# TUMFTM/RadarGNN

Measured on AMD Instinct MI355X. Metric: radar frames/sec (graph-build + GNN fwd), higher is better.
Workload: dtype f32 (dense layers: fp32 operands split into 2 f16 terms after an exact power-of-two pre-scale, 3 f16 MFMA products per fp32 product, fp32 accumulate -- more accurate than fp32 MFMA against float64, tests/test_gpu_f16x2.py; RGNN_NO_F16X2=1 selects 3 bf16 terms / 6 products, RGNN_LINEAR_FP32=1 v_mfma_; 1 GPU; C2: per GPU 64 RadarScenes-shaped frames x 3000 pts, radius graph r=1.0, node feats [rcs,velocity_vector,time_index,degree], edge feats [relative_position], 4-layer MPNNConv [224,224,128,64] + emb MLPs + both heads, train-mode BatchNorm, max aggr; frames_per_gpu=64, points_per_gpu=192000, edges_per_gpu=799078, ranks_in_process_group=1

## Files before the change

include/rgnn.h:

```cpp
#ifndef RGNN_H
#define RGNN_H

#include <stdint.h>

#ifdef __cplusplus
extern "C" {
#endif

typedef void* rgnn_stream_t;

#define RGNN_OK 0
#define RGNN_ERR_INVALID_ARGUMENT (-1)
#define RGNN_ERR_LAUNCH (-2)
#define RGNN_ERR_UNSUPPORTED (-3)

#define RGNN_STATUS_KNN_TOO_FEW_POINTS 1
#define RGNN_STATUS_DOT_PRODUCT 2
#define RGNN_STATUS_TIME_INDEX_OVERFLOW 4
#define RGNN_STATUS_EDGE_COUNT_CHANGED 8
#define RGNN_STATUS_NOT_SYMMETRIC 16
#define RGNN_STATUS_SPLITK_TIMEOUT 32
#define RGNN_STATUS_GT_OBJECT_TOO_LARGE 64
#define RGNN_STATUS_GT_DEGENERATE_OBJECT 128
#define RGNN_STATUS_PREPROCESS_BAD_ROW 256
// ... 144 lines not shown
  const float* residual; int64_t ldr;
  float* out; int64_t ldo;
  int64_t m; int32_t n;
  int32_t relu_out;
  float* col_stats;
  const int32_t* row_index;
  const int64_t* m_dev;
  int32_t accumulate;
  int32_t gather_only;
  const int32_t* residual_index;
  const void* W_planes;
  int32_t w_planes_kp;
  void* splitk_ws;
  int64_t splitk_ws_bytes;
  const float* a1_scale_shift;
  int32_t a1_relu;
  int32_t relu_from_col;
  const void* W_planes_f16;
  const float* a1_bound;
  const float* a2_bound;
  float* out_absmax;
  const int32_t* a1_panel_segment;
} rgnn_linear_args;
#define RGNN_BOUND_SLOTS 256
enum { RGNN_LINEAR_PATH_OTHER = 0, RGNN_LINEAR_PATH_DMA_BF16X3 = 1, RGNN_LINEAR_PATH_DMA_F16X2 = 2 };
int32_t rgnn_linear_fwd_path(const rgnn_linear_args* args );
int64_t rgnn_linear_planes_f16_bytes(int32_t n, int32_t k);
int rgnn_linear_split_weights_f16(const float* W1, const float* W2, int64_t ldw, int32_t w_split, int32_t n, int32_t k,
                                  void* planes , rgnn_stream_t stream);
int32_t rgnn_linear_fwd_fuses_a1_affine(const rgnn_linear_args* args );
enum { RGNN_LINEAR_FAMILY_NONE = 0, RGNN_LINEAR_FAMILY_TINY = 1, RGNN_LINEAR_FAMILY_FP32 = 2, RGNN_LINEAR_FAMILY_X3 = 3,
       RGNN_LINEAR_FAMILY_DMA = 4 };
void rgnn_linear_fwd_plan(const rgnn_linear_args* args , int32_t out[8] );
int64_t rgnn_linear_splitk_ws_bytes(void);
int64_t rgnn_linear_stat_panels(int64_t m);
int32_t rgnn_linear_planes_kp(int32_t k);
int rgnn_linear_split_weights(const float* W1, const float* W2, int64_t ldw, int32_t w_split, int32_t n, int32_t k,
                              void* planes , rgnn_stream_t stream);
int rgnn_linear_fwd(const rgnn_linear_args* args , rgnn_stream_t stream);

int32_t rgnn_embed3_supported(int32_t k0, int32_t n1, int32_t n2, int32_t n3);
int rgnn_embed3(const float* x, int64_t ldx, int32_t k0, const float* W1, int64_t ldw1, const float* b1, int32_t n1,
                const void* W2_planes_f16, const float* b2, int32_t n2, const void* W3_planes_f16, const float* b3, int32_t n3,
                int32_t relu3, int64_t m, float* out, int64_t ldo, float* out_absmax, rgnn_stream_t stream);
int rgnn_tiny_mlp2(const float* A, int64_t lda, int32_t k0, const int32_t* row_index , int64_t m,
                   const float* W1, int64_t ldw1, const float* b1, int32_t n1, int32_t relu1, const float* W2, int64_t ldw2,
                   const float* b2, int32_t n2, int32_t relu2, float* out, int64_t ldo, rgnn_stream_t stream);

int rgnn_batchnorm_finalize(const float* col_stats, int64_t panels, int64_t m, int32_t n, const float* gamma,
                            const float* beta, float* running_mean, float* running_var,
                            int64_t* num_batches_tracked, int32_t training, float momentum, float eps,
                            float* scale_shift , rgnn_stream_t stream);
int rgnn_batchnorm_finalize_parts(const float* stats_a, int64_t panels_a, const int64_t* rows_a ,
                                  const float* stats_b, int64_t panels_b, const int64_t* rows_b ,
                                  int64_t m, int32_t n, const float* gamma, const float* beta, float* running_mean,
                                  float* running_var, int64_t* num_batches_tracked, int32_t training, float momentum,
                                  float eps, float* scale_shift , rgnn_stream_t stream);
int rgnn_batchnorm_finalize_bound(const float* stats_a, int64_t panels_a, const int64_t* rows_a ,
                                  const float* stats_b, int64_t panels_b, const int64_t* rows_b ,
                                  int64_t m, int32_t n, const float* gamma, const float* beta, float* running_mean,
                                  float* running_var, int64_t* num_batches_tracked, int32_t training, float momentum,
                                  float eps, float* scale_shift , const float* in_bound, float* out_bound,
                                  rgnn_stream_t stream);
int rgnn_batchnorm_segments(const float* x, int64_t ldx, const int64_t* seg_ptr , int64_t n_seg, int32_t n,
                            const float* gamma, const float* beta, float* running_mean, float* running_var,
                            int64_t* num_batches_tracked, float momentum, float eps, double* seg_sums, float* table,
// ... 261 lines not shown
```

radargnn_amd/_lib.py:

```python
from __future__ import annotations

import ctypes as C
import os

import torch

_HERE = os.path.dirname(os.path.abspath(__file__))
LIB_PATH = os.environ.get("RGNN_LIB") or os.path.join(_HERE, "librgnn.so")

c_i32, c_i64, c_f32, c_f64, c_vp = C.c_int32, C.c_int64, C.c_float, C.c_double, C.c_void_p


class RgnnGrid(C.Structure):
    _fields_ = [("X", c_vp), ("dim", c_i32), ("n", c_i64), ("frame_ptr", c_vp), ("n_frames", c_i64),
                ("ws", c_vp), ("ws_bytes", c_i64)]


class RgnnLinearArgs(C.Structure):
    _fields_ = [("A1", c_vp), ("lda1", c_i64), ("k1", c_i32),
                ("A2", c_vp), ("lda2", c_i64), ("k2", c_i32),
                ("W1", c_vp), ("W2", c_vp), ("ldw", c_i64), ("w_split", c_i32),
                ("bias1", c_vp), ("bias2", c_vp),
                ("residual", c_vp), ("ldr", c_i64),
                ("out", c_vp), ("ldo", c_i64),
# ... 29 lines not shown
    "rgnn_radius_rows_commit": (c_i32, [c_vp, c_i64, c_i64, c_vp, c_vp, c_vp, c_vp, c_vp]),
    "rgnn_knn_graph": (c_i32, [C.POINTER(RgnnGrid), c_i32, c_vp, c_vp, c_vp, c_vp]),
    "rgnn_knn_graph_attrs": (c_i32, [C.POINTER(RgnnGrid), c_i32, c_vp, c_vp, c_vp, c_vp, c_i32, c_vp, c_vp]),
    "rgnn_knn_graph_frames": (c_i32, [C.POINTER(RgnnGrid), c_i32, c_i64, c_vp, c_vp, c_vp, c_vp, c_i32, c_vp, c_vp]),
    "rgnn_knn_degree_from_csr": (c_i32, [c_vp, c_vp, c_vp, c_vp, c_i64, c_i32, c_vp, c_vp]),
    "rgnn_undirected_degree_preset": (c_i32, [c_vp, c_vp, c_i64, c_vp, c_vp]),
    "rgnn_grid_cell_order": (c_i32, [C.POINTER(RgnnGrid), c_vp, c_vp]),
    "rgnn_undirected_degree": (c_i32, [c_vp, c_vp, c_i64, c_vp, c_vp, c_vp]),
    "rgnn_csr_by_target_tmp_bytes": (c_i64, [c_i64, c_i64]),
    "rgnn_invert_permutation": (c_i32, [c_vp, c_i64, c_vp, c_vp]),
    "rgnn_source_rowptr": (c_i32, [c_vp, c_i64, c_i64, c_vp, c_vp, c_vp, c_vp]),
    "rgnn_csr_by_target": (c_i32, [c_vp, c_i64, c_i64, c_vp, c_vp, c_vp, c_vp, c_vp, c_vp]),
    "rgnn_csr_by_target_unordered": (c_i32, [c_vp, c_i64, c_i64, c_vp, c_vp, c_vp, c_vp, c_vp, c_vp]),
    "rgnn_csr_by_target_frames": (c_i32, [c_vp, c_i64, c_i64, c_i64, c_vp, c_i64, c_i64, c_vp, c_vp, c_vp, c_vp, c_vp, c_vp, c_vp, c_vp]),
    "rgnn_csr_by_target_symmetric": (c_i32, [c_vp, c_vp, c_i64, c_i64, c_vp, c_vp, c_vp, c_vp, c_vp, c_vp, c_vp]),
    "rgnn_embed3_supported": (c_i32, [c_i32, c_i32, c_i32, c_i32]),
    "rgnn_embed3": (c_i32, [c_vp, c_i64, c_i32, c_vp, c_i64, c_vp, c_i32, c_vp, c_vp, c_i32, c_vp, c_vp, c_i32, c_i32, c_i64, c_vp, c_i64,
                            c_vp, c_vp]),
    "rgnn_csr_by_target_symmetric_own": (c_i32, [c_vp, c_vp, c_i64, c_i64, c_vp, c_vp, c_vp, c_vp, c_vp, c_vp, c_vp]),
    "rgnn_edge_features": (c_i32, [c_vp, c_vp, c_vp, c_i64, C.POINTER(c_i32), c_i32, c_i32, c_vp, c_i32, c_vp, c_vp]),
    "rgnn_edge_features_reversed": (c_i32, [c_vp, c_vp, c_vp, c_i64, c_vp, c_i64, C.POINTER(c_i32), c_i32, c_i32, c_vp, c_i32, c_vp, c_vp]),
    "rgnn_node_features": (c_i32, [c_vp, c_vp, c_vp, c_vp, c_vp, c_i64, C.POINTER(c_i32), c_i32, c_vp, c_i32, c_vp]),
    "rgnn_node_features_time_index": (c_i32, [c_vp, c_vp, c_vp, c_vp, c_vp, c_i64, c_vp, c_i64, C.POINTER(c_i32), c_i32, c_vp, c_i32,
                                              c_vp, c_vp, c_vp]),
    "rgnn_split_by_degree_frames": (c_i32, [c_vp, c_vp, c_i64, c_vp, c_vp, c_vp, c_vp, c_vp, c_vp, c_vp]),
    "rgnn_radius_counts": (c_i32, [c_vp, c_i64, c_vp, c_i32, c_vp, c_vp]),
    "rgnn_time_index": (c_i32, [c_vp, c_vp, c_i64, c_vp, c_vp, c_vp]),
    "rgnn_time_index_ws_bytes": (c_i64, [c_i64]),
    "rgnn_time_index_ws": (c_i32, [c_vp, c_vp, c_i64, c_i64, c_vp, c_vp, c_vp, c_i64, c_vp]),
    "rgnn_linear_stat_panels": (c_i64, [c_i64]),
    "rgnn_linear_fwd": (c_i32, [C.POINTER(RgnnLinearArgs), c_vp]),
    "rgnn_linear_fwd_fuses_a1_affine": (c_i32, [C.POINTER(RgnnLinearArgs)]),
    "rgnn_linear_fwd_plan": (None, [C.POINTER(RgnnLinearArgs), C.POINTER(c_i32 * 8)]),
    "rgnn_linear_planes_kp": (c_i32, [c_i32]),
    "rgnn_linear_fwd_path": (c_i32, [C.POINTER(RgnnLinearArgs)]),
    "rgnn_linear_planes_f16_bytes": (c_i64, [c_i32, c_i32]),
    "rgnn_linear_split_weights_f16": (c_i32, [c_vp, c_vp, c_i64, c_i32, c_i32, c_i32, c_vp, c_vp]),
    "rgnn_linear_splitk_ws_bytes": (c_i64, []),
    "rgnn_linear_split_weights": (c_i32, [c_vp, c_vp, c_i64, c_i32, c_i32, c_i32, c_vp, c_vp]),
    "rgnn_tiny_mlp2": (c_i32, [c_vp, c_i64, c_i32, c_vp, c_i64, c_vp, c_i64, c_vp, c_i32, c_i32, c_vp, c_i64, c_vp, c_i32, c_i32, c_vp,
                       c_i64, c_vp]),
    "rgnn_batchnorm_finalize": (c_i32, [c_vp, c_i64, c_i64, c_i32, c_vp, c_vp, c_vp, c_vp, c_vp, c_i32, c_f32, c_f32,
                                        c_vp, c_vp]),
    "rgnn_batchnorm_finalize_parts": (c_i32, [c_vp, c_i64, c_vp, c_vp, c_i64, c_vp, c_i64, c_i32, c_vp, c_vp, c_vp, c_vp, c_vp, c_i32,
                                              c_f32, c_f32, c_vp, c_vp]),
    "rgnn_batchnorm_finalize_bound": (c_i32, [c_vp, c_i64, c_vp, c_vp, c_i64, c_vp, c_i64, c_i32, c_vp, c_vp, c_vp, c_vp, c_vp, c_i32,
                                              c_f32, c_f32, c_vp, c_vp, c_vp, c_vp]),
    "rgnn_batchnorm_segments": (c_i32, [c_vp, c_i64, c_vp, c_i64, c_i32, c_vp, c_vp, c_vp, c_vp, c_vp, c_f32, c_f32, c_vp, c_vp,
                                        c_vp, c_vp, c_vp]),
    "rgnn_batchnorm_act_segments": (c_i32, [c_vp, c_i64, c_vp, c_i64, c_i32, c_vp, c_vp, c_vp, c_vp, c_vp, c_f32, c_f32, c_i32, c_vp,
                                            c_vp, c_vp, c_i64, c_vp, c_vp, c_vp]),
    "rgnn_batchnorm_segments_from_panels": (c_i32, [c_vp, c_vp, c_vp, c_vp, c_vp, c_i64, c_i32, c_vp, c_vp, c_vp, c_vp, c_vp, c_f32,
                                                    c_f32, c_vp, c_vp, c_vp, c_vp, c_vp]),
    "rgnn_pad_list_by_segment": (c_i32, [c_vp, c_vp, c_vp, c_i64, c_vp, c_vp, c_vp, c_vp, c_vp]),
    "rgnn_pad_list_pair_by_segment": (c_i32, [c_vp, c_vp, c_vp, c_vp, c_vp, c_i64, c_vp, c_vp, c_vp, c_vp, c_vp, c_vp, c_vp, c_vp, c_vp]),
    "rgnn_scale_shift_act_segments": (c_i32, [c_vp, c_i64, c_vp, c_vp, c_i64, c_i64, c_i32, c_i32, c_vp, c_i64, c_vp]),
    "rgnn_column_stats": (c_i32, [c_vp, c_i64, c_i64, c_i32, c_vp, c_vp]),
    "rgnn_scale_shift_act": (c_i32, [c_vp, c_i64, c_vp, c_i64, c_i32, c_i32, c_vp, c_i64, c_vp]),
    "rgnn_mpnn_aggregate": (c_i32, [c_vp, c_i64, c_vp, c_vp, c_i64, c_vp, c_i64, c_vp, c_i32, c_vp, c_vp, c_vp, c_vp, c_i32,
                                    c_i64, c_i32, c_i32, c_vp, c_i64, c_vp]),
    "rgnn_mpnn_aggregate_flags": (c_i32, [c_vp, c_i64, c_vp, c_vp, c_i64, c_vp, c_i64, c_vp, c_i32, c_vp, c_vp, c_vp, c_vp, c_i32,
                                          c_i64, c_i32, c_i32, c_vp, c_i64, c_i32, c_vp]),
    "rgnn_mpnn_aggregate_absmax": (c_i32, [c_vp, c_i64, c_vp, c_vp, c_i64, c_vp, c_i64, c_vp, c_i32, c_vp, c_vp, c_vp, c_vp, c_i32,
                                           c_i64, c_i32, c_i32, c_vp, c_i64, c_i32, c_vp, c_vp]),
    "rgnn_mpnn_aggregate_max_arg": (c_i32, [c_vp, c_vp, c_i64, c_vp, c_i64, c_vp, c_i32, c_vp, c_vp, c_vp, c_vp, c_i32, c_i64, c_i32,
                                             c_vp, c_i64, c_vp, c_i32, C.POINTER(c_i32), c_vp]),
# ... 118 lines not shown
```

radargnn_amd/csrc/linear.hip:

```cpp
#include "linear_common.h"

namespace {


template <bool VEC, bool IDX>
__device__ __forceinline__ float4 load_a(const LinParams& p, int64_t M, int64_t gm, int64_t row, int gk) {
  const int K = p.k1 + p.k2;
  if (VEC) {
    const bool ok = (gm < M) && (gk < K);
    const int64_t r = row;
    const int k = (gk < K) ? gk : (K - 4);
    const float* ptr = (k < p.k1) ? (p.A1 + r * p.lda1 + k) : (p.A2 + r * p.lda2 + (k - p.k1));
    float4 v = *(const float4*)ptr;
    if (!ok) v = make_float4(0.f, 0.f, 0.f, 0.f);
    return v;
  } else {
    float4 v = make_float4(0.f, 0.f, 0.f, 0.f);
    if (gm >= M) return v;
    float t[4];
#pragma unroll
    for (int j = 0; j < 4; j++) {
      const int k = gk + j;
      t[j] = (k < K) ? ((k < p.k1) ? p.A1[row * p.lda1 + k] : p.A2[row * p.lda2 + (k - p.k1)]) : 0.f;
    }
// ... 759 lines not shown
    }
    if (vec4) {
#pragma unroll
      for (int c = 0; c < 16; c += 4)
        if (c < n2) *(float4*)(out + r * ldo + c) = make_float4(o[c], o[c + 1], o[c + 2], o[c + 3]);
    } else {
#pragma unroll
      for (int c = 0; c < 16; c++)
        if (c < n2) out[r * ldo + c] = o[c];
    }
  }
}

inline bool aligned16(const void* ptr) { return ((uintptr_t)ptr & 15) == 0; }

}

extern "C" int rgnn_tiny_mlp2(const float* A, int64_t lda, int32_t k0, const int32_t* row_index, int64_t m, const float* W1,
                              int64_t ldw1, const float* b1, int32_t n1, int32_t relu1, const float* W2, int64_t ldw2,
                              const float* b2, int32_t n2, int32_t relu2, float* out, int64_t ldo, rgnn_stream_t stream) {
  RGNN_CHECK_ARG(m >= 0 && k0 >= 1 && k0 <= 8 && n1 >= 1 && n1 <= 8 && n2 >= 1 && n2 <= 16, "widths: <= 8 in, <= 8 hidden, <= 16 out");
  if (m == 0) return RGNN_OK;
  RGNN_CHECK_ARG(A && W1 && W2 && out, "null pointers");
  const int vec4 = (n2 % 4 == 0) && (ldo % 4 == 0) && aligned16(out);
  const int64_t blocks = rgnn_blocks(m, 256) < 8192 ? rgnn_blocks(m, 256) : 8192;
  hipLaunchKernelGGL(k_tiny_mlp2, dim3((unsigned)blocks), dim3(256), 0, (hipStream_t)stream, A, lda, k0, row_index, m, W1, ldw1, b1, n1,
                     relu1, W2, ldw2, b2, n2, relu2, out, ldo, vec4);
  RGNN_CHECK_LAUNCH();
  return RGNN_OK;
}

int rgnn_linear_dma_tile(int n, int64_t m, int f16_form, int* lds_bytes);
void rgnn_linear_dma_launch(const void* lin_params, int tn, int subset, hipStream_t s);

struct LinearPlan {
  int family = RGNN_LINEAR_FAMILY_NONE;
  int form = RGNN_LINEAR_PATH_OTHER;
  bool vec = false;
  bool bufl = false;
  bool direct_epilogue = false, fast_epilogue = false;
  bool x3_subset = false;
  int ext_a1 = 0, ext_a2 = 0, ext_w = 0, ext_out = 0, ext_wp = 0;
  int tile_cols = 0, nt = 0;
  int tn = 0;
  bool split_k = false;
  bool no_split_k = false;
  int stagger = 100;
  int lds_bytes = 0;
  bool affine_batch = false;
  bool affine_segments = false;
};

static LinearPlan plan_linear(const rgnn_linear_args* a) {
  LinearPlan pl;
  if (a == nullptr || a->m <= 0 || a->n <= 0 || a->k1 < 0 || a->k2 < 0 || a->k1 + a->k2 <= 0 || !a->out || !a->W1 ||
      (a->k1 > 0 && !a->A1) || (a->k2 > 0 && !a->A2) || (a->w_split < a->n && !a->W2))
    return pl;
  const int k = a->k1 + a->k2;
  const bool one_w = a->w_split >= a->n;
  pl.vec = (a->k1 % 4 == 0) && (a->k2 % 4 == 0) && (a->ldw % 4 == 0) && aligned16(a->W1) &&
           (a->W2 == nullptr || aligned16(a->W2)) &&
           (a->k1 == 0 || (a->lda1 % 4 == 0 && aligned16(a->A1))) &&
           (a->k2 == 0 || (a->lda2 % 4 == 0 && aligned16(a->A2)));
  const int64_t e1 = a->k1 ? ((a->m - 1) * a->lda1 + a->k1) * 4 : 0;
  const int64_t e2 = a->k2 ? ((a->m - 1) * a->lda2 + a->k2) * 4 : 0;
  const int64_t ew = ((int64_t)(a->n - 1) * a->ldw + k) * 4;
  const int64_t eo = ((a->m - 1) * a->ldo + a->n) * 4;
  const int64_t lim = ((int64_t)1 << 31) - 64;
  pl.bufl = pl.vec && a->k1 > 0 && one_w && e1 < lim && e2 < lim && ew < lim && (a->k2 == 0 || a->k1 % BK == 0) &&
            RGNN_ENV("RGNN_LINEAR_NO_BUFL") == nullptr;
  pl.ext_a1 = (int)e1; pl.ext_a2 = (int)e2; pl.ext_w = (int)ew; pl.ext_out = (int)(eo < lim ? eo : 0);
  pl.fast_epilogue = (a->n % 4 == 0) && (a->ldo % 4 == 0) && aligned16(a->out) &&
                     (a->residual == nullptr || (a->ldr % 4 == 0 && aligned16(a->residual))) &&
                     (a->bias1 == nullptr || aligned16(a->bias1)) && (a->bias2 == nullptr || aligned16(a->bias2)) &&
                     (one_w || a->w_split % 4 == 0);
  pl.direct_epilogue = a->row_index == nullptr && a->residual == nullptr && eo < lim && RGNN_ENV("RGNN_LINEAR_NO_DIRECT") == nullptr;
  const bool no_affine = RGNN_ENV("RGNN_DMA_NO_AFFINE") != nullptr;

  if (a->k2 == 0 && a->k1 <= 8 && a->n <= 64 && one_w && a->residual == nullptr && a->row_index == nullptr &&
      a->col_stats == nullptr && a->m >= 4096 && a->relu_from_col <= 0 && RGNN_ENV("RGNN_LINEAR_NO_TINY") == nullptr) {
    pl.family = RGNN_LINEAR_FAMILY_TINY;
    return pl;
  }

  const bool subset = a->row_index != nullptr && !a->accumulate && !a->gather_only && a->residual == nullptr && eo < lim &&
                      a->relu_from_col <= 0;
  if (a->W_planes && pl.bufl && (pl.direct_epilogue || subset) && a->w_planes_kp >= k && a->w_planes_kp % BK == 0 &&
      (int64_t)3 * a->n * a->w_planes_kp * 2 < lim && RGNN_ENV("RGNN_LINEAR_FP32") == nullptr) {
    pl.x3_subset = subset;
    pl.form = RGNN_LINEAR_PATH_DMA_BF16X3;
    pl.ext_wp = (int)((int64_t)3 * a->n * a->w_planes_kp * 2);
    const int dma_min_n = RGNN_ENV("RGNN_DMA_MIN_N") ? atoi(RGNN_ENV("RGNN_DMA_MIN_N")) : 32;
    if (a->n > dma_min_n && k % 16 == 0 && a->k1 % 16 == 0 && RGNN_ENV("RGNN_X3_NODMA") == nullptr) {
      pl.family = RGNN_LINEAR_FAMILY_DMA;
      if (a->W_planes_f16 != nullptr && a->a1_bound != nullptr && (a->k2 == 0 || a->a2_bound != nullptr) &&
          RGNN_ENV("RGNN_LINEAR_NO_F16") == nullptr) {
        pl.form = RGNN_LINEAR_PATH_DMA_F16X2;
        pl.ext_wp = (int)((int64_t)2 * a->n * a->w_planes_kp * 2);
      }
      pl.tn = rgnn_linear_dma_tile(a->n, a->m, pl.form == RGNN_LINEAR_PATH_DMA_F16X2, &pl.lds_bytes);
      pl.tile_cols = 32 * pl.tn; pl.nt = (a->n + pl.tile_cols - 1) / pl.tile_cols;
      pl.split_k = a->splitk_ws && a->splitk_ws_bytes >= rgnn_linear_splitk_ws_bytes() && RGNN_ENV("RGNN_DMA_NOSK") == nullptr;
      pl.no_split_k = RGNN_ENV("RGNN_DMA_NOPSK") != nullptr;
      pl.stagger = RGNN_ENV("RGNN_DMA_STAGGER") ? atoi(RGNN_ENV("RGNN_DMA_STAGGER")) : 100;
      const int64_t table = RGNN_AFFINE_ROWS * 4 * (int64_t)a->k1;
      pl.affine_batch = !no_affine && pl.lds_bytes + table <= LDS_BYTES;
      pl.affine_segments = !no_affine && subset && a->k1 <= 512 && pl.lds_bytes + 2 * table <= LDS_BYTES;
      return pl;
    }
    pl.family = RGNN_LINEAR_FAMILY_X3;
    const int pad_w = (a->n + 255) / 256 * 256, pad_n = (a->n + 127) / 128 * 128;
    const bool wide = a->n > 128 && pad_w * 100 <= pad_n * 107 && RGNN_ENV("RGNN_X3_NARROW") == nullptr;
    pl.tile_cols = wide ? 256 : a->n > 64 ? 128 : a->n > 32 ? 64 : 32;
    pl.nt = (a->n + pl.tile_cols - 1) / pl.tile_cols;
    return pl;
  }

  pl.family = RGNN_LINEAR_FAMILY_FP32;
  if (pl.bufl && a->row_index == nullptr && a->n > 128 && a->n <= 512 && k >= 192) {
    const int base = ((a->n + 127) / 128) * 128;
    int best = base;
    for (int tn = 3; tn <= 7; tn++) {
      const int w = 32 * tn, padded = ((a->n + w - 1) / w) * w;
      if (padded < best || (padded == best && pl.tn)) { best = padded; pl.tn = tn; }
    }
    if (best * 100 > base * 95) pl.tn = 0;
  }
  pl.tile_cols = pl.tn ? 32 * pl.tn : a->n > 64 ? 128 : a->n > 32 ? 64 : 32;
  pl.nt = (a->n + pl.tile_cols - 1) / pl.tile_cols;
  const bool planes_keep_separate_pass = a->W_planes != nullptr;
  pl.affine_batch = !no_affine && pl.bufl && !planes_keep_separate_pass;
  return pl;
}

extern "C" int32_t rgnn_linear_fwd_path(const rgnn_linear_args* a) {
  const LinearPlan pl = plan_linear(a);
  return pl.family == RGNN_LINEAR_FAMILY_DMA ? pl.form : RGNN_LINEAR_PATH_OTHER;
}

static bool applies_a1_affine(const LinearPlan& pl, const rgnn_linear_args* a) {
  return a->a1_panel_segment != nullptr ? pl.affine_segments : pl.affine_batch;
}
extern "C" int32_t rgnn_linear_fwd_fuses_a1_affine(const rgnn_linear_args* a) {
  return a != nullptr && applies_a1_affine(plan_linear(a), a) ? 1 : 0;
}

extern "C" void rgnn_linear_fwd_plan(const rgnn_linear_args* a, int32_t out[8]) {
  const LinearPlan pl = plan_linear(a);
  out[0] = pl.family; out[1] = pl.form; out[2] = pl.tile_cols; out[3] = pl.nt;
  out[4] = pl.x3_subset; out[5] = pl.bufl; out[6] = a != nullptr && applies_a1_affine(pl, a); out[7] = pl.split_k;
}

extern "C" int64_t rgnn_linear_stat_panels(int64_t m) { return (m + BM - 1) / BM; }
extern "C" int64_t rgnn_linear_splitk_ws_bytes(void) { return (int64_t)256 * 8 * 16 * 512 * 4 + 4096; }

extern "C" int rgnn_linear_fwd(const rgnn_linear_args* a, rgnn_stream_t stream) {
  RGNN_CHECK_ARG(a != nullptr, "null args");
  RGNN_CHECK_ARG(a->m >= 0 && a->n >= 0 && a->k1 >= 0 && a->k2 >= 0, "negative sizes");
  if (a->m == 0 || a->n == 0) return RGNN_OK;
  RGNN_CHECK_ARG(a->k1 + a->k2 > 0, "empty reduction dimension");
  RGNN_CHECK_ARG(a->out && a->W1 && (a->k1 == 0 || a->A1) && (a->k2 == 0 || a->A2), "null pointers");
  RGNN_CHECK_ARG(a->w_split >= a->n || a->W2, "w_split < n needs W2");
  RGNN_CHECK_ARG(a->m < ((int64_t)1 << 31) * BM, "m too large");
  RGNN_CHECK_ARG(a->a1_panel_segment == nullptr || a->a1_scale_shift != nullptr, "a1_panel_segment needs a1_scale_shift");
  const LinearPlan pl = plan_linear(a);
  if (a->out_absmax != nullptr && pl.family != RGNN_LINEAR_FAMILY_DMA) {
    rgnn_set_error("rgnn_linear_fwd: out_absmax needs the LDS-DMA kernel (rgnn_linear_fwd_path != 0)");
    return RGNN_ERR_UNSUPPORTED;
  }
  if (a->a1_scale_shift != nullptr && !applies_a1_affine(pl, a)) {
    rgnn_set_error("rgnn_linear_fwd: a1_scale_shift needs the LDS-DMA kernel (rgnn_linear_fwd_fuses_a1_affine): apply "
                   "rgnn_scale_shift_act to A1 instead");
    return RGNN_ERR_UNSUPPORTED;
  }
  RGNN_CHECK_ARG(a->row_index != nullptr || (a->m_dev == nullptr && a->accumulate == 0), "m_dev / accumulate need row_index");
  RGNN_CHECK_ARG(!(a->accumulate && a->col_stats), "col_stats of an accumulating launch are not defined (statistics are sums about a pivot of the stored values)");
  hipStream_t s = (hipStream_t)stream;
  if (pl.family == RGNN_LINEAR_FAMILY_TINY) {
    const bool v4 = (a->n % 4 == 0) && (a->ldo % 4 == 0) && aligned16(a->out);
    const int64_t threads = a->m * ((a->n + 3) / 4);
    const int64_t tiny_blocks = rgnn_blocks(threads, 256) < 4096 ? rgnn_blocks(threads, 256) : 4096;
    rgnn_prof_begin(s);
    hipLaunchKernelGGL(v4 ? k_linear_tiny<true> : k_linear_tiny<false>, dim3((unsigned)tiny_blocks), dim3(256), 0, s, (const float*)a->A1,
                       a->lda1, a->k1, (const float*)a->W1, a->ldw, (const float*)a->bias1, a->m, a->n, a->relu_out, (float*)a->out, a->ldo);
    rgnn_prof_end(s);
    RGNN_CHECK_LAUNCH();
    return RGNN_OK;
  }
  const bool f16 = pl.family == RGNN_LINEAR_FAMILY_DMA && pl.form == RGNN_LINEAR_PATH_DMA_F16X2;
  LinParams p;
  p.A1 = a->A1; p.A2 = a->A2; p.lda1 = a->lda1; p.lda2 = a->lda2; p.k1 = a->k1; p.k2 = a->k2;
  p.W1 = a->W1; p.W2 = a->W2; p.ldw = a->ldw; p.w_split = a->w_split >= a->n ? a->n : a->w_split;
  p.bias1 = a->bias1; p.bias2 = a->bias2; p.residual = a->residual; p.ldr = a->ldr;
  p.out = a->out; p.ldo = a->ldo; p.m = a->m; p.n = a->n; p.relu_out = a->relu_out; p.col_stats = a->col_stats;
  p.mt = (int)((a->m + BM - 1) / BM); p.nt = pl.nt;
  p.ext_a1 = pl.ext_a1; p.ext_a2 = pl.ext_a2; p.ext_w = pl.ext_w;
  p.row_index = a->row_index; p.m_dev = a->m_dev; p.gather_only = a->gather_only; p.res_index = a->residual_index; p.accumulate = a->accumulate;
  p.fast_epilogue = pl.fast_epilogue; p.direct_epilogue = pl.direct_epilogue; p.ext_out = pl.ext_out;
  p.Wp = f16 ? a->W_planes_f16 : a->W_planes; p.kp = a->w_planes_kp; p.ext_wp = pl.ext_wp;
  p.sk_ws = pl.split_k ? a->splitk_ws : nullptr;
  p.sk_flags = pl.split_k ? (int*)((char*)a->splitk_ws + (int64_t)256 * 8 * 16 * 512 * 4) : nullptr;
  p.no_split_k = pl.no_split_k; p.stagger = pl.stagger;
  p.a1_aff = a->a1_scale_shift; p.a1_relu = a->a1_relu; p.a1_aff_panel = a->a1_panel_segment;
  p.relu_lo = a->relu_from_col > 0 ? a->relu_from_col : 0;
  p.fmt = f16 ? 1 : 0; p.a1_bound = a->a1_bound; p.a2_bound = a->a2_bound; p.out_absmax = a->out_absmax;
  rgnn_prof_begin(s);
  if (pl.family == RGNN_LINEAR_FAMILY_DMA) {
    rgnn_linear_dma_launch(&p, pl.tn, pl.x3_subset, s);
  } else if (pl.family == RGNN_LINEAR_FAMILY_X3) {
#define RGNN_X3(IDX)                                                                         \
  do {                                                                                       \
    if (pl.tile_cols == 256) launch_x3<IDX, 256, 256, 2, 4, 4, 2, 16, 1>(p, s);              \
    else if (pl.tile_cols == 128) launch_x3<IDX, 256, 128, 4, 2, 2, 2>(p, s);                \
    else if (pl.tile_cols == 64) launch_x3<IDX, 256, 64, 4, 2, 2, 1>(p, s);                  \
    else launch_x3<IDX, 256, 32, 8, 1, 1, 1>(p, s);                                          \
  } while (0)
    if (pl.x3_subset) RGNN_X3(true); else RGNN_X3(false);
#undef RGNN_X3
  } else if (pl.tn) {
    switch (pl.tn) {
      case 3: launch<96, 4, 1, 1, 3, 1, true>(p, pl.vec, pl.bufl, s); break;
      case 4: launch<128, 4, 1, 1, 4, 1, true>(p, pl.vec, pl.bufl, s); break;
      case 5: launch<160, 4, 1, 1, 5, 1, true>(p, pl.vec, pl.bufl, s); break;
      case 6: launch<192, 4, 1, 1, 6, 1, true>(p, pl.vec, pl.bufl, s); break;
      default: launch<224, 4, 1, 1, 7, 1, true>(p, pl.vec, pl.bufl, s); break;
    }
  } else if (pl.tile_cols == 128) {
    launch<128, 2, 2, 2, 2>(p, pl.vec, pl.bufl, s);
  } else if (pl.tile_cols == 64) {
    launch<64, 2, 2, 2, 1>(p, pl.vec, pl.bufl, s);
  } else {
    launch<32, 4, 1, 1, 1>(p, pl.vec, pl.bufl, s);
  }
  rgnn_prof_end(s);
  RGNN_CHECK_LAUNCH();
  return RGNN_OK;
}

extern "C" int32_t rgnn_linear_planes_kp(int32_t k) { return (k + BK - 1) / BK * BK; }

// ... 33 lines not shown
```

radargnn_amd/csrc/linear_dma.hip:

```cpp
#include "linear_common.h"

namespace {

typedef int i32x4 __attribute__((ext_vector_type(4)));

__device__ __forceinline__ void dma16(i32x4 rsrc, int voff, int soff, unsigned lds_base) {
  asm volatile(
      "s_mov_b32 m0, %3\n\t"
      "s_nop 0\n\t"
      "buffer_load_dwordx4 %0, %1, %2 offen lds"
      :
      : "v"(voff), "s"(rsrc), "s"(soff), "s"(lds_base)
      : "memory");
}
template <int N>
__device__ __forceinline__ void dma_wait() {
  asm volatile("s_waitcnt vmcnt(%0)" ::"i"(N) : "memory");
}

__device__ __forceinline__ i32x4 make_rsrc(const void* base, int bytes) {
  const uint64_t a = (uint64_t)base;
  i32x4 r;
  r.x = __builtin_amdgcn_readfirstlane((int)(uint32_t)a);
  r.y = __builtin_amdgcn_readfirstlane((int)(uint32_t)((a >> 32) & 0xffff));
// ... 528 lines not shown
    for (int o = 32; o > 0; o >>= 1) amax = fmaxf(amax, __shfl_xor(amax, o, 64));
    __syncthreads();
    if (lane == 0) stat_lds[wave] = amax;
    __syncthreads();
    if (t == 0) {
      float m = stat_lds[0];
#pragma unroll
      for (int w = 1; w < WV; w++) m = fmaxf(m, stat_lds[w]);
      bound_raise(p.out_absmax, blockIdx.x, m);
    }
  }
}

template <int TN, bool IDX, int FMT, int WV = 8>
void launch_dma(LinParams p, hipStream_t s) {
  constexpr int BN = 32 * TN;
  constexpr int NPL = FMT ? 2 : 3;
  constexpr int DMA_BM = 32 * WV, DMA_THREADS = 64 * WV;
  const size_t lds = (size_t)dma_lds_bytes(BN, NPL, WV) + (p.a1_aff ? (size_t)(p.a1_aff_panel ? 2 : 1) * RGNN_AFFINE_ROWS * 4 * p.k1 : 0);
  p.nt = (p.n + BN - 1) / BN;
  p.mt = (int)((p.m + DMA_BM - 1) / DMA_BM);
  const int64_t tiles = (int64_t)p.mt * p.nt;
  int64_t grid = 256 * (8 / WV);
  if (grid > tiles && (TN > 4 || p.sk_ws == nullptr || p.no_split_k || 2 * tiles > grid)) grid = tiles;
  grid = (grid + 7) / 8 * 8;
  static RgnnOncePerDevice attr_once;
  if (attr_once.first()) {
    const int most = dma_lds_bytes(BN, NPL, WV) + 12288 < LDS_BYTES ? dma_lds_bytes(BN, NPL, WV) + 12288 : LDS_BYTES;
    hipFuncSetAttribute((const void*)k_linear_dma<TN, IDX, FMT, WV>, hipFuncAttributeMaxDynamicSharedMemorySize, most);
  }
  hipLaunchKernelGGL((k_linear_dma<TN, IDX, FMT, WV>), dim3((unsigned)grid), dim3(DMA_THREADS), lds, s, p);
}

}

static int dma_pick_tn(int n, int64_t m, int npl) {
  const int top = npl == 3 ? 7 : 8;
  const char* e = RGNN_ENV("RGNN_DMA_TN");
  if (e) { const int v = atoi(e); if (v >= 2 && v <= top) return v; }
  int best = 2;
  if (n > 64 && n <= 96) best = 3;
  if (n > 96) {
    best = top;
    int best_pad = (n + 32 * top - 1) / (32 * top) * (32 * top);
    for (int tn = top - 1; tn >= 3; tn--) {
      const int w = 32 * tn, pad = (n + w - 1) / w * w;
      if (pad < best_pad) { best_pad = pad; best = tn; }
    }
  }
  const int64_t mt = (m + DMA_BM_MAX - 1) / DMA_BM_MAX;
  if (mt * ((n + 32 * best - 1) / (32 * best)) >= 192 || RGNN_ENV("RGNN_DMA_NO_SMALL_M")) return best;
  double best_t = 1e30;
  int pick = best;
  for (int tn = 2; tn <= top; tn++) {
    const int64_t tiles = mt * ((n + 32 * tn - 1) / (32 * tn));
    const double t = (double)((tiles + 255) / 256) * (0.35 + 0.2 * tn);
    if (t < best_t - 1e-9) { best_t = t; pick = tn; }
  }
  return pick;
}

static bool dma_four_waves(const LinParams& p, int tn, int waves_env) {
  if (waves_env == 4) return true;
  if (waves_env == 8) return false;
  (void)tn;
  return false;
}

int rgnn_linear_dma_tile(int n, int64_t m, int f16_form, int* lds_bytes) {
  const int npl = f16_form ? 2 : 3;
  const int tn = dma_pick_tn(n, m, npl);
  *lds_bytes = dma_lds_bytes(32 * tn, npl);
  return tn;
}

void rgnn_linear_dma_launch(const void* params, int tn, int subset, hipStream_t s) {
  const LinParams& p = *(const LinParams*)params;
  const char* waves_e = RGNN_ENV("RGNN_DMA_WAVES");
  const int waves_env = waves_e ? atoi(waves_e) : 0;
  const bool four = p.fmt == 1 && p.a1_aff_panel == nullptr && dma_four_waves(p, tn, waves_env);
#define RGNN_DMA(TN)                                                                                     \
  case TN:                                                                                               \
    if (four) { if (subset) launch_dma<TN, true, 1, 4>(p, s); else launch_dma<TN, false, 1, 4>(p, s); }  \
    else if (p.fmt == 1) { if (subset) launch_dma<TN, true, 1>(p, s); else launch_dma<TN, false, 1>(p, s); }  \
    else { if (subset) launch_dma<TN, true, 0>(p, s); else launch_dma<TN, false, 0>(p, s); }             \
    break
  switch (tn) {
    RGNN_DMA(2); RGNN_DMA(3); RGNN_DMA(4); RGNN_DMA(5); RGNN_DMA(6); RGNN_DMA(7);
    default:
      if (four) { if (subset) launch_dma<8, true, 1, 4>(p, s); else launch_dma<8, false, 1, 4>(p, s); }
      else if (p.fmt == 1) { if (subset) launch_dma<8, true, 1>(p, s); else launch_dma<8, false, 1>(p, s); }
      else { if (subset) launch_dma<8, true, 0>(p, s); else launch_dma<8, false, 0>(p, s); }
  }
#undef RGNN_DMA
}
```

Measured before the change: 33020 frames/s.

## Add panel-resident DMA linear kernel that keeps A rows in registers across column tiles

Adds a new schedule for the f16x2 DMA linear path. It applies when K≤128, there is no second operand, no column-stat output, and at least 192 row panels. Each 512-thread block loads a 256-row A panel once, pre-splits it into f16 hi/lo registers (applying the scale or the fused affine+ReLU), then walks all column tiles while streaming double-buffered weight slabs through LDS. This avoids re-reading and re-splitting A for every N tile, as the ring schedule does. The cost is high register pressure, a fixed TN=2 tile width and a fixed 256-block grid with a hand-rolled partial-panel split across XCD slots.

After: 33530 frames/s, median of 6. 1.02x the previous value.

```diff
diff --git a/include/rgnn.h b/include/rgnn.h
--- a/include/rgnn.h
+++ b/include/rgnn.h
@@ -200,6 +200,9 @@
 enum { RGNN_LINEAR_FAMILY_NONE = 0, RGNN_LINEAR_FAMILY_TINY = 1, RGNN_LINEAR_FAMILY_FP32 = 2, RGNN_LINEAR_FAMILY_X3 = 3,
        RGNN_LINEAR_FAMILY_DMA = 4 };
 void rgnn_linear_fwd_plan(const rgnn_linear_args* args , int32_t out[8] );
+enum { RGNN_LINEAR_SCHEDULE_RING = 0, RGNN_LINEAR_SCHEDULE_PANEL = 1 };
+#define RGNN_LINEAR_PANEL_MIN_PANELS 192
+int32_t rgnn_linear_fwd_schedule(const rgnn_linear_args* args );
 int64_t rgnn_linear_splitk_ws_bytes(void);
 int64_t rgnn_linear_stat_panels(int64_t m);
 int32_t rgnn_linear_planes_kp(int32_t k);
diff --git a/radargnn_amd/_lib.py b/radargnn_amd/_lib.py
--- a/radargnn_amd/_lib.py
+++ b/radargnn_amd/_lib.py
@@ -85,6 +85,7 @@
     "rgnn_linear_fwd": (c_i32, [C.POINTER(RgnnLinearArgs), c_vp]),
     "rgnn_linear_fwd_fuses_a1_affine": (c_i32, [C.POINTER(RgnnLinearArgs)]),
     "rgnn_linear_fwd_plan": (None, [C.POINTER(RgnnLinearArgs), C.POINTER(c_i32 * 8)]),
+    "rgnn_linear_fwd_schedule": (c_i32, [C.POINTER(RgnnLinearArgs)]),
     "rgnn_linear_planes_kp": (c_i32, [c_i32]),
     "rgnn_linear_fwd_path": (c_i32, [C.POINTER(RgnnLinearArgs)]),
     "rgnn_linear_planes_f16_bytes": (c_i64, [c_i32, c_i32]),
diff --git a/radargnn_amd/csrc/linear.hip b/radargnn_amd/csrc/linear.hip
--- a/radargnn_amd/csrc/linear.hip
+++ b/radargnn_amd/csrc/linear.hip
@@ -815,6 +815,8 @@
 
 int rgnn_linear_dma_tile(int n, int64_t m, int f16_form, int* lds_bytes);
 void rgnn_linear_dma_launch(const void* lin_params, int tn, int subset, hipStream_t s);
+int rgnn_linear_panel_fits(int n, int k, int with_table);
+void rgnn_linear_panel_launch(const void* lin_params, int subset, hipStream_t s);
 
 struct LinearPlan {
   int family = RGNN_LINEAR_FAMILY_NONE;
@@ -832,6 +834,7 @@
   int lds_bytes = 0;
   bool affine_batch = false;
   bool affine_segments = false;
+  bool panel = false;
 };
 
 static LinearPlan plan_linear(const rgnn_linear_args* a) {
@@ -889,6 +892,10 @@
       const int64_t table = RGNN_AFFINE_ROWS * 4 * (int64_t)a->k1;
       pl.affine_batch = !no_affine && pl.lds_bytes + table <= LDS_BYTES;
       pl.affine_segments = !no_affine && subset && a->k1 <= 512 && pl.lds_bytes + 2 * table <= LDS_BYTES;
+      pl.panel = pl.form == RGNN_LINEAR_PATH_DMA_F16X2 && a->k2 == 0 && k <= 128 && a->col_stats == nullptr &&
+                 a->a1_panel_segment == nullptr && (a->m + 255) / 256 >= RGNN_LINEAR_PANEL_MIN_PANELS &&
+                 (a->a1_scale_shift == nullptr || !no_affine) && rgnn_linear_panel_fits(a->n, k, a->a1_scale_shift != nullptr) &&
+                 RGNN_ENV("RGNN_DMA_NO_PANEL") == nullptr;
       return pl;
     }
     pl.family = RGNN_LINEAR_FAMILY_X3;
@@ -932,6 +939,10 @@
   const LinearPlan pl = plan_linear(a);
   out[0] = pl.family; out[1] = pl.form; out[2] = pl.tile_cols; out[3] = pl.nt;
   out[4] = pl.x3_subset; out[5] = pl.bufl; out[6] = a != nullptr && applies_a1_affine(pl, a); out[7] = pl.split_k;
+}
+
+extern "C" int32_t rgnn_linear_fwd_schedule(const rgnn_linear_args* a) {
+  return plan_linear(a).panel ? RGNN_LINEAR_SCHEDULE_PANEL : RGNN_LINEAR_SCHEDULE_RING;
 }
 
 extern "C" int64_t rgnn_linear_stat_panels(int64_t m) { return (m + BM - 1) / BM; }
@@ -988,7 +999,9 @@
   p.relu_lo = a->relu_from_col > 0 ? a->relu_from_col : 0;
   p.fmt = f16 ? 1 : 0; p.a1_bound = a->a1_bound; p.a2_bound = a->a2_bound; p.out_absmax = a->out_absmax;
   rgnn_prof_begin(s);
-  if (pl.family == RGNN_LINEAR_FAMILY_DMA) {
+  if (pl.family == RGNN_LINEAR_FAMILY_DMA && pl.panel) {
+    rgnn_linear_panel_launch(&p, pl.x3_subset, s);
+  } else if (pl.family == RGNN_LINEAR_FAMILY_DMA) {
     rgnn_linear_dma_launch(&p, pl.tn, pl.x3_subset, s);
   } else if (pl.family == RGNN_LINEAR_FAMILY_X3) {
 #define RGNN_X3(IDX)                                                                         \
diff --git a/radargnn_amd/csrc/linear_dma.hip b/radargnn_amd/csrc/linear_dma.hip
--- a/radargnn_amd/csrc/linear_dma.hip
+++ b/radargnn_amd/csrc/linear_dma.hip
@@ -584,6 +584,257 @@
   hipLaunchKernelGGL((k_linear_dma<TN, IDX, FMT, WV>), dim3((unsigned)grid), dim3(DMA_THREADS), lds, s, p);
 }
 
+constexpr int PNL_TN = 2;
+constexpr int PNL_D = 2;
+constexpr int PNL_A_SUB = DMA_BM_MAX * DMA_BK * 4;
+__host__ __device__ constexpr int pnl_slab_bytes(int kb) { return kb * 2 * (32 * PNL_TN) * 32; }
+__host__ __device__ constexpr int pnl_lds_fixed(int kb) { return 2 * pnl_slab_bytes(kb) + PNL_D * PNL_A_SUB + 16 * 4 + DMA_BM_MAX * 4; }
+constexpr int PNL_KB = 8;
+
+template <int KB, bool IDX>
+__global__ __launch_bounds__(512) void k_linear_panel(const LinParams p) {
+  constexpr int TN = PNL_TN, BN = 32 * TN, WV = 8, BMT = DMA_BM_MAX, THREADS = 64 * WV;
+  constexpr int SLAB = pnl_slab_bytes(KB);
+  constexpr int NF = SLAB / PNL_A_SUB, NS = PNL_D + NF;
+  constexpr int NWS = KB / 2;
+  constexpr int NST = TN * 16;
+  static_assert(KB % 2 == 0 && NS >= 2 && NS <= KB && NST < 64, "panel-resident config");
+  extern __shared__ __attribute__((aligned(16))) float smem[];
+  char* const lds = (char*)smem;
+  float* const xch = (float*)(lds + 2 * SLAB + PNL_D * PNL_A_SUB);
+  int* const row_tab = (int*)(xch + 16);
+  float* const bias_lds = (float*)(row_tab + BMT);
+  float* const aff_lds = bias_lds + p.nt * BN;
+  const unsigned lds0 = (unsigned)(uintptr_t)(__attribute__((address_space(3))) char*)lds;
+
+  const int64_t M = (IDX && p.m_dev) ? *p.m_dev : p.m;
+  const int mt = (int)((M + BMT - 1) / BMT);
+  const int xcd = blockIdx.x & 7, slot = blockIdx.x >> 3, g8 = gridDim.x >> 3;
+  const int my_panels = (mt > xcd) ? (mt - xcd + 7) / 8 : 0;
+  const int t = threadIdx.x, lane = t & 63;
+  const int wave = __builtin_amdgcn_readfirstlane(t >> 6);
+  const int K = p.k1;
+  const int nkb = K / DMA_BK;
+  const int full = my_panels / g8, rem = my_panels - full * g8;
+  int cut = 0;
+  if (rem > 0) { cut = g8 / rem; if (cut > p.nt) cut = p.nt; }
+  const bool tail = rem > 0 && slot < rem * cut;
+  const int n_mine = full + (tail ? 1 : 0);
+  if (n_mine == 0) return;
+  if (p.stagger > 0 && full > 0) {
+    const float period_us = (float)nkb * 0.16f + 2.2f * TN;
+    const int unit = (int)(0.8f * period_us * (float)p.stagger * 0.01f);
+    const int units = (slot & 31) * (unit > 0 ? unit : 1);
+    for (int u = 0; u < units; u++) __builtin_amdgcn_s_sleep(1);
+  }
+  const i32x4 ra1_d = make_rsrc(p.A1, p.ext_a1);
+  const i32x4 rw_d = make_rsrc(p.Wp, p.ext_wp);
+
+  float a_mul, out_mul;
+  {
+    float bound = bound_read(p.a1_bound);
+    bound = __builtin_bit_cast(float, __builtin_amdgcn_readfirstlane(__builtin_bit_cast(int, bound)));
+    const int be = (int)((__float_as_uint(bound) >> 23) & 255u);
+    int se = 268 - be;
+    se = se > 253 ? 253 : se;
+    a_mul = __uint_as_float((unsigned)se << 23);
+    const float* foot = (const float*)((const char*)p.Wp + (size_t)2 * p.n * p.kp * 2);
+    out_mul = __uint_as_float((unsigned)(254 - se) << 23) * foot[2];
+  }
+  const bool aff_on = p.a1_aff != nullptr;
+  const float aff_lo = p.a1_relu ? 0.f : -INFINITY;
+  if (aff_on)
+    for (int i = t; i < RGNN_AFFINE_ROWS * p.k1; i += THREADS) aff_lds[i] = i < p.k1 ? p.a1_aff[i] : p.a1_aff[i] * a_mul;
+  for (int gn = t; gn < p.nt * BN; gn += THREADS) {
+    float b = 0.f;
+    if (gn < p.n) {
+      const float* bp = (gn < p.w_split) ? p.bias1 : p.bias2;
+      if (bp) b = bp[(gn < p.w_split) ? gn : gn - p.w_split];
+    }
+    bias_lds[gn] = b;
+  }
+  __syncthreads();
+
+  int va1[2];
+  auto a_offsets = [&](int panel) {
+    const int64_t m0 = (int64_t)panel * BMT + wave * 32;
+    const int left = M - m0 > 32 ? 32 : (int)(M - m0);
+    const int lda4 = (int)p.lda1 * 4;
+#pragma unroll
+    for (int s = 0; s < 2; s++) {
+      const int r = 16 * s + (lane >> 2);
+      int row = -1;
+      if (r < left) row = IDX ? p.row_index[m0 + r] : (int)m0 + r;
+      const int c = ((lane & 3) ^ ((r >> 2) & 3)) * 16;
+      va1[s] = (row >= 0) ? row * lda4 + c : OOB;
+    }
+  };
+  auto stage_off = [&](int i, int fb) -> int { return i < PNL_D ? 2 * SLAB + i * PNL_A_SUB : fb * SLAB + (i - PNL_D) * PNL_A_SUB; };
+  auto issue_a = [&](int kb, int off) {
+    const int kill = kb < nkb ? 0 : OOB;
+    const int soff = __builtin_amdgcn_readfirstlane(kb * DMA_BK * 4);
+    const unsigned base = __builtin_amdgcn_readfirstlane(lds0 + off + wave * 2048);
+    dma16(ra1_d, va1[0] | kill, soff, base);
+    dma16(ra1_d, va1[1] | kill, soff, base + 1024);
+  };
+  const int w_row = (t >> 1) & (BN - 1);
+  const int vw0 = (((t >> 8) * 2 + ((t >> 7) & 1)) * p.n + w_row) * 32 + (((t & 1) ^ ((w_row >> 3) & 1)) * 16);
+  auto slab_request = [&](int ct, int buf) {
+    const int vw = ct * BN + w_row < p.n ? vw0 + ct * (BN * 32) : OOB;
+#pragma unroll
+    for (int s = 0; s < NWS; s++) {
+      const int kill = 2 * s + (wave >> 2) < nkb ? 0 : OOB;
+      const int soff = __builtin_amdgcn_readfirstlane(2 * s * 2 * p.n * 32);
+      const unsigned base = __builtin_amdgcn_readfirstlane(lds0 + buf * SLAB + s * (THREADS * 16) + wave * 1024);
+      dma16(rw_d, vw | kill, soff, base);
+    }
+  };
+
+  const int ga = (lane >> 2) & 3;
+  const int a_off0 = wave * 2048 + (lane & 31) * 64 + (((2 * (lane >> 5)) ^ ga) * 16);
+  const int a_off1 = a_off0 ^ 16;
+  const int b_off = (lane & 31) * 32 + (((lane >> 5) ^ ((lane >> 3) & 1)) * 16);
+  auto split_a = [&](float4 x0, float4 x1, int kb, raw16x8& h, raw16x8& l) {
+    if (aff_on) {
+      const float* mu = aff_lds + kb * DMA_BK + 8 * (lane >> 5);
+      const float* sc = mu + p.k1;
+      const float* sh = sc + p.k1;
+      typedef float f32x2 __attribute__((ext_vector_type(2)));
+      const float4 m0 = *(const float4*)mu, m1 = *(const float4*)(mu + 4);
+      const float4 s0 = *(const float4*)sc, s1 = *(const float4*)(sc + 4), t0 = *(const float4*)sh, t1 = *(const float4*)(sh + 4);
+      const f32x2 y0 = __builtin_elementwise_fma(f32x2{x0.x, x0.y} - f32x2{m0.x, m0.y}, f32x2{s0.x, s0.y}, f32x2{t0.x, t0.y});
+      const f32x2 y1 = __builtin_elementwise_fma(f32x2{x0.z, x0.w} - f32x2{m0.z, m0.w}, f32x2{s0.z, s0.w}, f32x2{t0.z, t0.w});
+      const f32x2 y2 = __builtin_elementwise_fma(f32x2{x1.x, x1.y} - f32x2{m1.x, m1.y}, f32x2{s1.x, s1.y}, f32x2{t1.x, t1.y});
+      const f32x2 y3 = __builtin_elementwise_fma(f32x2{x1.z, x1.w} - f32x2{m1.z, m1.w}, f32x2{s1.z, s1.w}, f32x2{t1.z, t1.w});
+      x0.x = fmaxf(y0.x, aff_lo); x0.y = fmaxf(y0.y, aff_lo); x0.z = fmaxf(y1.x, aff_lo); x0.w = fmaxf(y1.y, aff_lo);
+      x1.x = fmaxf(y2.x, aff_lo); x1.y = fmaxf(y2.y, aff_lo); x1.z = fmaxf(y3.x, aff_lo); x1.w = fmaxf(y3.y, aff_lo);
+    } else {
+      x0.x *= a_mul; x0.y *= a_mul; x0.z *= a_mul; x0.w *= a_mul;
+      x1.x *= a_mul; x1.y *= a_mul; x1.z *= a_mul; x1.w *= a_mul;
+    }
+    f16x4_t h0, l0, h1, l1;
+    split2(x0, h0, l0);
+    split2(x1, h1, l1);
+    h = __builtin_bit_cast(raw16x8, __builtin_shufflevector(h0, h1, 0, 1, 2, 3, 4, 5, 6, 7));
+    l = __builtin_bit_cast(raw16x8, __builtin_shufflevector(l0, l1, 0, 1, 2, 3, 4, 5, 6, 7));
+  };
+  auto mm = [&](const raw16x8& a, const raw16x8& b, const f32x16& c) -> f32x16 {
+    return __builtin_amdgcn_mfma_f32_32x32x16_f16(__builtin_bit_cast(f16x8_t, a), __builtin_bit_cast(f16x8_t, b), c, 0, 0, 0);
+  };
+
+  raw16x8 ah[KB], al[KB];
+  f32x16 acc[1][TN];
+  float amax = 0.f;
+  int wb = 0;
+  for (int j = 0; j < n_mine; j++) {
+    int pl_, c_lo = 0, c_hi = p.nt;
+    if (j < full) {
+      pl_ = slot + j * g8;
+    } else {
+      const int part = slot % cut;
+      pl_ = full * g8 + slot / cut;
+      c_lo = p.nt * part / cut; c_hi = p.nt * (part + 1) / cut;
+    }
+    const int panel = xcd + 8 * pl_;
+    __syncthreads();
+    slab_request(c_lo, wb);
+    a_offsets(panel);
+#pragma unroll
+    for (int i = 0; i < NS; i++) issue_a(i, stage_off(i, wb ^ 1));
+#pragma unroll
+    for (int kb = 0; kb < KB; kb++) {
+      if (KB - 1 - kb >= NS - 1) dma_wait<2 * (NS - 1)>();
+      else if (KB - 1 - kb == 3) dma_wait<6>();
+      else if (KB - 1 - kb == 2) dma_wait<4>();
+      else if (KB - 1 - kb == 1) dma_wait<2>();
+      else dma_wait<0>();
+      const int off = stage_off(kb % NS, wb ^ 1);
+      if (kb < nkb) {
+        const float4 x0 = *(const float4*)(lds + off + a_off0), x1 = *(const float4*)(lds + off + a_off1);
+        split_a(x0, x1, kb, ah[kb], al[kb]);
+      }
+#if defined(__HIP_DEVICE_COMPILE__)
+      asm volatile("" :: "v"(ah[kb]), "v"(al[kb]));
+#endif
+      if (kb + NS < KB) issue_a(kb + NS, off);
+    }
+    for (int ct = c_lo; ct < c_hi; ct++) {
+      if (ct > c_lo) dma_wait<NST>();
+      __builtin_amdgcn_s_barrier();
+#if defined(__HIP_DEVICE_COMPILE__)
+      asm volatile("" ::: "memory");
+#endif
+      if (ct + 1 < c_hi) slab_request(ct + 1, wb ^ 1);
+      float bias_r[TN];
+#pragma unroll
+      for (int jn = 0; jn < TN; jn++) bias_r[jn] = bias_lds[ct * BN + jn * 32 + (lane & 31)];
+#pragma unroll
+      for (int jn = 0; jn < TN; jn++)
+#pragma unroll
+        for (int r = 0; r < 16; r++) acc[0][jn][r] = 0.f;
+      const char* st = lds + wb * SLAB + b_off;
+      auto read_b = [&](int kb, int pl, raw16x8 (&b)[TN]) {
+#pragma unroll
+        for (int jn = 0; jn < TN; jn++) b[jn] = *(const raw16x8*)(st + kb * (2 * BN * 32) + pl * (BN * 32) + jn * 1024);
+      };
+      raw16x8 bh[2][TN], bl[TN];
+      auto read_1 = [&](int kb, int pl, int jn, raw16x8& b) { b = *(const raw16x8*)(st + kb * (2 * BN * 32) + pl * (BN * 32) + jn * 1024); };
+      auto block = [&](int kb, bool more) {
+        const int c = kb & 1;
+        if (more) read_1(kb + 1, 0, 0, bh[c ^ 1][0]);
+        acc[0][0] = mm(al[kb], bh[c][0], acc[0][0]); acc[0][1] = mm(al[kb], bh[0][1], acc[0][1]);
+        acc[0][0] = mm(ah[kb], bl[0], acc[0][0]); acc[0][1] = mm(ah[kb], bl[1], acc[0][1]);
+        if (more) read_b(kb + 1, 1, bl);
+        acc[0][0] = mm(ah[kb], bh[c][0], acc[0][0]); acc[0][1] = mm(ah[kb], bh[0][1], acc[0][1]);
+        if (more) read_1(kb + 1, 0, 1, bh[0][1]);
+      };
+      read_1(0, 0, 0, bh[0][0]); read_1(0, 0, 1, bh[0][1]);
+      read_b(0, 1, bl);
+      if (nkb == KB) {
+#pragma unroll
+        for (int kb = 0; kb < KB; kb++) block(kb, kb + 1 < KB);
+      } else {
+#pragma unroll
+        for (int kb = 0; kb < KB; kb++)
+          if (kb < nkb) block(kb, kb + 1 < nkb);
+      }
+      amax = direct_epilogue<BN, WV, 1, 1, TN, BMT, IDX, true>(p, acc, (int64_t)panel * BMT, ct * BN, panel, M, xch, row_tab, bias_r,
+                                                                out_mul, amax);
+      wb ^= 1;
+    }
+  }
+  dma_wait<0>();
+  if (p.out_absmax) {
+    int ln = lane;
+#if defined(__HIP_DEVICE_COMPILE__)
+    asm volatile("" : "+v"(ln));
+#endif
+#pragma unroll
+    for (int o = 32; o > 0; o >>= 1)
+      amax = fmaxf(amax, __int_as_float(__builtin_amdgcn_ds_bpermute((ln ^ o) << 2, __float_as_int(amax))));
+    __syncthreads();
+    if (lane == 0) xch[wave] = amax;
+    __syncthreads();
+    if (t == 0) {
+      float m = xch[0];
+#pragma unroll
+      for (int w = 1; w < WV; w++) m = fmaxf(m, xch[w]);
+      bound_raise(p.out_absmax, blockIdx.x, m);
+    }
+  }
+}
+
+template <int KB, bool IDX>
+void launch_panel(LinParams p, hipStream_t s) {
+  p.nt = (p.n + 32 * PNL_TN - 1) / (32 * PNL_TN);
+  p.mt = (int)((p.m + DMA_BM_MAX - 1) / DMA_BM_MAX);
+  const size_t lds = (size_t)pnl_lds_fixed(KB) + (size_t)p.nt * 32 * PNL_TN * 4 + (p.a1_aff ? (size_t)RGNN_AFFINE_ROWS * 4 * p.k1 : 0);
+  static RgnnOncePerDevice attr_once;
+  if (attr_once.first())
+    hipFuncSetAttribute((const void*)k_linear_panel<KB, IDX>, hipFuncAttributeMaxDynamicSharedMemorySize, LDS_BYTES);
+  hipLaunchKernelGGL((k_linear_panel<KB, IDX>), dim3(256), dim3(512), lds, s, p);
+}
+
 }
 
 static int dma_pick_tn(int n, int64_t m, int npl) {
@@ -646,3 +897,13 @@
   }
 #undef RGNN_DMA
 }
+
+int rgnn_linear_panel_fits(int n, int k, int with_table) {
+  const int nt = (n + 32 * PNL_TN - 1) / (32 * PNL_TN);
+  return k <= PNL_KB * DMA_BK && (int64_t)pnl_lds_fixed(PNL_KB) + (int64_t)nt * 32 * PNL_TN * 4 + (with_table ? (int64_t)RGNN_AFFINE_ROWS * 4 * k : 0) <= LDS_BYTES;
+}
+
+void rgnn_linear_panel_launch(const void* params, int subset, hipStream_t s) {
+  const LinParams& p = *(const LinParams*)params;
+  if (subset) launch_panel<PNL_KB, true>(p, s); else launch_panel<PNL_KB, false>(p, s);
+}
```
